# fenghansen/YOND_public

Measured on AMD Instinct MI355X. Metric: Bayer megapixels/sec end-to-end (NLE+VST+denoise+iVST), higher is better.
Workload: dtype f32 (3x3 convolutions: f32 operands as two f16 halves -- 22-23 significant bits -- on the f16 MFMA, 3 products per f32 product, f32 accumulate; per-layer error vs float64 asserted <= 2x the f32 direct kernel's and <= 2e-5 of max|ref| (tests/test_hip_conv.py; measured 1.3e-6 vs 1.5e-6), whole frame v

## Files before the change

include/yond_hip.h:

```cpp
#ifndef YOND_HIP_H
#define YOND_HIP_H

#include <stddef.h>
#include <stdint.h>

#ifdef __cplusplus
extern "C" {
#endif

#define YOND_OK 0
#define YOND_EINVAL (-1)
#define YOND_EUNSUPPORTED (-2)

#define YOND_ABI_VERSION 8
int yond_abi_version(void);

int yond_pack_vst_norm_f32(const float* bayer, int H, int W, float* out, int pad_l, int pad_r, int pad_t,
                           int pad_b, int mode, double scale, double gain, double sigma, double lo,
                           double hi, const double* lut_x, const float* lut_y, int lut_n, float* img_max,
                           void* stream);

int yond_pack_vst_norm_biaslut_f32(const float* bayer, int H, int W, float* out, int pad_l, int pad_r, int pad_t,
                                   int pad_b, double scale, double gain, double sigma, double lo, double hi,
                                   const double* lut_x, const double* lut_y, int lut_n, float* img_max, void* stream);
// ... 28 lines not shown
typedef struct YondConvDesc {
    const float* src0;
    const float* src1;
    int C0, C1;
    int N, H, W;
    int Ho, Wo;
    int Cout;
    int ksize;
    int stride;
    int shuffle;
    int pre_act;
    int post_act;
    float slope;
    const float* wpk;
    const float* escale;
    const float* eshift;
    int ebatch;
    const float* res;
    float* dst;
    int tn;
    int kc;
    int algo;
    const float* out4_w;
    const float* out4_b;
    const float* out4_x;
    const float* out4_ub;
    float* out4_dst;
    unsigned int* status;
    int in_fmt, out_fmt;
    int res_fmt;
    unsigned long long* clk;
    int tile_order;
    float* dst2;
} YondConvDesc;
#define YOND_STATUS_HALF_OVERFLOW 1u
#define YOND_FMT_NHWC_F32 0
#define YOND_FMT_SPLIT_PLANES 1
#define YOND_FMT_PLANES4 2
#define YOND_SP_PLANE_UNITS(H, W) ((((H) * (W)) + 8) / 8 * 8)
#define YOND_SP_BYTES(N, C, H, W) ((size_t)(N) * ((C) / 16) * 4 * (size_t)YOND_SP_PLANE_UNITS(H, W) * 16)
#define YOND_HP_BYTES(N, C, H, W) ((size_t)(N) * ((C) / 16) * 2 * (size_t)YOND_SP_PLANE_UNITS(H, W) * 16)

int yond_conv_config(int ksize, int stride, int cin, int cout, int shuffle, int N, int Ho, int Wo, int* tn, int* kc);
int yond_pack_conv_weight_f32(const float* w, int cout, int cin, int ksize, int tn, int kc, float* dst);
int yond_pack_conv_weight_split_f32(const float* w, int cout, int cin, int ksize, int tn, int kc, float* dst);
int yond_conv2d_f32(const YondConvDesc* desc, void* stream);

int yond_conv_wino_supported(int cin, int cout);
int yond_pack_conv_wino_weight_f32(const float* w, int cout, int cin, int tn, float* dst);

int yond_conv_split_supported(int ksize, int stride, int cin, int cout);
int yond_pack_conv_split_weight_f32(const float* w, int cout, int cin, int ksize, int tn, int parts, float* dst);
int yond_gemm_k1_stationary_supported(const YondConvDesc* desc);
int yond_pack_conv_split_weight_dev_f32(const float* w, int cout, int cin, int ksize, int tn, int parts, float* dst, int* status,
                                        void* stream);
int yond_pack_conv_split_weights_batch_dev_f32(const float* src, const long long* desc, int nlayers, float* dst, size_t ngroups,
                                               int* status, void* stream);

int yond_conv_in_f32(const float* x, const float* ub , int N, int H, int W, int Cout,
                     const float* wpk, const float* bias, float slope, float* dst,
                     int out_fmt , void* stream);
int yond_pack_conv_in_weight_f32(const float* w , int cout, float* dst );

int yond_conv_out_f32(const float* feat , int Cin, const float* w ,
                      const float* bias , const float* x ,
                      const float* ub , int N, int H, int W, float* dst ,
                      void* stream);

int yond_maxpool2_f32(const float* src, int N, int H, int W, int C, float* dst, void* stream);

typedef struct YondFilmDesc {
    int kind, C, ld;
    const float *w_a0, *b_a0, *w_a2, *b_a2;
    const float *w_b0, *b_b0;
    const float *w_b, *b_b;
    const float *cb1, *cb2;
    float *s1, *t1, *s2, *t2;
} YondFilmDesc;
int yond_film_f32(const YondFilmDesc* descs, int nblocks, const float* t , const float* ub ,
                  int N, void* stream);

int yond_box_stats_self1_f32(const float* bayer, int H, int W, int k, int k2, int tile_w, float* mean,
                             float* var, float* blur2, void* stream);
int yond_box_stats_self2_f32(const float* blur2, int h, int w, int k, int tile_w, float* lap, void* stream);
int yond_box_stats_collab_f32(const float* bayer_lr, const float* bayer_hr, int H, int W, int k, int tile_w,
                              float* mean, float* var, float* lap, void* stream);


int yond_box_stats_self_stats_f32(const float* bayer, int H, int W, int k, int k2, int tile_w, float* mean, float* var,
                                  float* blur2, float* lap, const double* q_host, int nq, void* ws, void* stream);
int yond_box_stats_collab_stats_f32(const float* bayer_lr, const float* bayer_hr, int H, int W, int k, int tile_w,
                                    float* mean, float* var, float* lap, const double* q_host, int nq, void* ws, void* stream);

size_t yond_select_ws_bytes(int nr);
int yond_select_ranks_f32(const float* data, size_t n, const int64_t* ranks_host, int nr, float* out, void* ws,
                          void* stream);
int yond_percentiles_f32(const float* data, size_t n, const double* q_host, int nq, double* out, void* ws,
                         void* stream);

size_t yond_nle_ws_bytes(size_t n);
int yond_nle_stats_f32(const float* lap, const float* mean, size_t n, int width, const double* q_host, int nq, void* ws,
                       void* stream);
int yond_nle_threshold_f32(const float* lap, size_t n, const double* q_host, int nq, int want_score, void* ws, void* stream);
int yond_nle_state_layout(int* off );
int yond_nle_moments_f32(const float* lap, const float* mean, const float* var, size_t n, void* ws, void* stream);

// ... 214 lines not shown
```

yond_public_amd/_lib.py:

```python
import ctypes as C
import os

import torch

_HERE = os.path.dirname(os.path.abspath(__file__))
LIB_PATH = os.environ.get("YOND_HIP_LIB", os.path.join(_HERE, "libyond_hip.so"))
_lib = None
ABI_VERSION = 8

vp, i32, f32, f64, sz, i64 = C.c_void_p, C.c_int, C.c_float, C.c_double, C.c_size_t, C.c_longlong


class YondConvDesc(C.Structure):
    _fields_ = [("src0", vp), ("src1", vp), ("C0", i32), ("C1", i32), ("N", i32), ("H", i32), ("W", i32),
                ("Ho", i32), ("Wo", i32), ("Cout", i32), ("ksize", i32), ("stride", i32), ("shuffle", i32),
                ("pre_act", i32), ("post_act", i32), ("slope", f32), ("wpk", vp), ("escale", vp),
                ("eshift", vp), ("ebatch", i32), ("res", vp), ("dst", vp), ("tn", i32), ("kc", i32), ("algo", i32),
                ("out4_w", vp), ("out4_b", vp), ("out4_x", vp), ("out4_ub", vp), ("out4_dst", vp), ("status", vp),
                ("in_fmt", i32), ("out_fmt", i32), ("res_fmt", i32), ("clk", vp), ("tile_order", i32), ("dst2", vp)]


class YondBlock0Desc(C.Structure):
    _fields_ = [("x", vp), ("in_fmt", i32), ("N", i32), ("H", i32), ("W", i32), ("w1", vp), ("w2", vp),
                ("s1", vp), ("t1", vp), ("s2", vp), ("t2", vp), ("ebatch", i32), ("dst", vp),
                ("out4_w", vp), ("out4_b", vp), ("out4_x", vp), ("out4_ub", vp), ("out4_dst", vp), ("status", vp)]


class YondFilmDesc(C.Structure):
    _fields_ = [("kind", i32), ("C", i32), ("ld", i32),
                ("w_a0", vp), ("b_a0", vp), ("w_a2", vp), ("b_a2", vp), ("w_b0", vp), ("b_b0", vp),
                ("w_b", vp), ("b_b", vp), ("cb1", vp), ("cb2", vp),
                ("s1", vp), ("t1", vp), ("s2", vp), ("t2", vp)]


PROTOTYPES = {
    "yond_abi_version": [],
    "yond_pack_vst_norm_f32": [vp, i32, i32, vp, i32, i32, i32, i32, i32, f64, f64, f64, f64, f64, vp, vp, i32, vp, vp],
    "yond_pack_vst_norm_biaslut_f32": [vp, i32, i32, vp, i32, i32, i32, i32, f64, f64, f64, f64, f64, vp, vp, i32, vp, vp],
    "yond_bias_eval_f32": [vp, sz, vp, vp, i32, i32, i32, f64, f64, vp, vp],
    "yond_denorm_ivst_unpack_f32": [vp, i32, i32, i32, i32, i32, i32, vp, i32, f64, f64, f64, f64, f64, i32, vp],
    "yond_pack_vst_norm_batch_f32": [vp, i32, i32, i32, vp, i32, i32, i32, i32, f64, f64, f64, f64, f64, vp, vp, i32, i32, vp, vp],
    "yond_denorm_ivst_unpack_batch_f32": [vp, i32, i32, i32, i32, i32, i32, i32, vp, i32, f64, f64, f64, f64, f64, i32, vp],
    "yond_vst_elem_f32": [vp, sz, f64, f64, f64, vp, vp],
    "yond_ivst_elem_f64": [vp, sz, f64, f64, i32, vp, vp],
    "yond_bayer2rggb_f32": [vp, i32, i32, vp, vp],
    "yond_rggb2bayer_f32": [vp, i32, i32, vp, vp],
    "yond_rot90_f32": [vp, i32, i32, i32, i32, vp, vp],
    "yond_nchw4_to_nhwc4_f32": [vp, vp, i32, i32, i32, vp],
    "yond_nhwc4_to_nchw4_f32": [vp, vp, i32, i32, i32, vp],
    "yond_image_max_f32": [vp, i32, sz, vp, vp, vp],
    "yond_conv_config": [i32, i32, i32, i32, i32, i32, i32, i32, C.POINTER(i32), C.POINTER(i32)],
    "yond_pack_conv_weight_f32": [vp, i32, i32, i32, i32, i32, vp],
    "yond_conv2d_f32": [C.POINTER(YondConvDesc), vp],
    "yond_conv_wino_supported": [i32, i32],
    "yond_pack_conv_wino_weight_f32": [vp, i32, i32, i32, vp],
    "yond_pack_conv_weight_split_f32": [vp, i32, i32, i32, i32, i32, vp],
    "yond_conv_split_supported": [i32, i32, i32, i32],
    "yond_pack_conv_split_weight_f32": [vp, i32, i32, i32, i32, i32, vp],
    "yond_gemm_k1_stationary_supported": [C.POINTER(YondConvDesc)],
    "yond_pack_conv_split_weight_dev_f32": [vp, i32, i32, i32, i32, i32, vp, vp, vp],
    "yond_pack_conv_split_weights_batch_dev_f32": [vp, vp, i32, vp, sz, vp, vp],
    "yond_conv_in_f32": [vp, vp, i32, i32, i32, i32, vp, vp, f32, vp, i32, vp],
    "yond_pack_conv_in_weight_f32": [vp, i32, vp],
    "yond_conv_out_f32": [vp, i32, vp, vp, vp, vp, i32, i32, i32, vp, vp],
    "yond_maxpool2_f32": [vp, i32, i32, i32, i32, vp, vp],
    "yond_film_f32": [vp, i32, vp, vp, i32, vp],
    "yond_box_stats_self1_f32": [vp, i32, i32, i32, i32, i32, vp, vp, vp, vp],
    "yond_box_stats_self2_f32": [vp, i32, i32, i32, i32, vp, vp],
    "yond_box_stats_collab_f32": [vp, vp, i32, i32, i32, i32, vp, vp, vp, vp],
    "yond_box_stats_self_stats_f32": [vp, i32, i32, i32, i32, i32, vp, vp, vp, vp, vp, i32, vp, vp],
    "yond_box_stats_collab_stats_f32": [vp, vp, i32, i32, i32, i32, vp, vp, vp, vp, i32, vp, vp],
    "yond_select_ws_bytes": [i32],
    "yond_select_ranks_f32": [vp, sz, vp, i32, vp, vp, vp],
    "yond_percentiles_f32": [vp, sz, vp, i32, vp, vp, vp],
    "yond_nle_ws_bytes": [sz],
    "yond_nle_stats_f32": [vp, vp, sz, i32, vp, i32, vp, vp],
    "yond_nle_threshold_f32": [vp, sz, vp, i32, i32, vp, vp],
    "yond_nle_state_layout": [vp],
    "yond_nle_moments_f32": [vp, vp, vp, sz, vp, vp],
    "yond_nlf_occupancy_f32": [vp, vp, sz, i32, vp, i32, vp, vp],
    "yond_nlf_score3_f64": [vp, vp, vp, i32, vp, vp, vp],
    "yond_nlf_moments_f32": [vp, vp, vp, sz, vp, vp, vp],
    "yond_bias_lut_f64": [vp, i32, f64, f64, vp, vp],
    "yond_block_metrics_tiles": [i32, i32],
    "yond_block_metrics_f32": [vp, vp, i32, i32, i32, i32, vp, vp],
    "yond_block_metrics_rgb8": [vp, vp, i32, i32, i32, i32, vp, vp],
    "yond_render_srgb": [vp, i32, i32, i32, i32, i32, C.POINTER(f64), C.POINTER(f64), i32, vp, vp, i32, vp, f64, vp],
    "yond_clock_probe": [f64, vp, vp],
    "yond_img2raw_f32": [vp, sz, i32, i32, i32, vp, vp, i32, i32, i32, vp, vp, vp, vp],
    "yond_pg_noise_f32": [vp, vp, sz, i32, vp, i32, vp],
    "yond_camera_noise_f32": [vp, vp, sz, i32, vp, i32, i32, vp],
    "yond_est_conv_in_f32": [vp, i32, i32, i32, i32, vp, vp, vp, vp],
    "yond_est_head_f32": [vp, i32, i32, i32, i32, vp, vp, i32, i32, i32, vp, vp, vp],
    "yond_est_head_ws_bytes": [i32, i32],
    "yond_conv_wgrad_f32": [vp, vp, i32, i32, i32, i32, i32, i32, i32, i32, i32, vp, vp],
    "yond_conv_wgrad_ws_f32": [vp, vp, i32, i32, i32, i32, i32, i32, i32, i32, i32, vp, vp, sz, vp],
    "yond_conv_wgrad_ws_bytes": [i32, i32, i32, i32, i32, i32, i32, i32, i32],
    "yond_conv_wgrad_split_ws_bytes": [i32, i32, i32, i32, i32],
    "yond_conv_wgrad_split_f32": [vp, vp, i32, i32, i32, i32, i32, vp, i32, vp, sz, vp, vp],
    "yond_colsum_f32": [vp, sz, i32, vp, vp],
    "yond_film_silu_supported": [i32],
    "yond_film_silu_f32": [vp, vp, vp, vp, i32, sz, i32, vp],
    "yond_film_silu_bwd_f32": [vp, vp, vp, vp, vp, vp, vp, i32, sz, i32, vp],
    "yond_film_mlp_fwd_f32": [vp, vp, vp, vp, vp, vp, vp, i32, i32, i32, vp, vp, vp],
    "yond_film_mlp_bwd_f32": [vp, vp, vp, vp, vp, vp, vp, vp, i32, i32, i32, vp, vp, vp, vp, vp, vp, vp, vp],
    "yond_film_mlp_fwd_multi_f32": [vp, i32, vp],
    "yond_gemm_split_f32": [vp, i32, sz, i32, i32, i64, i64, i32, vp, vp, i32, i32, i32, i32, vp, vp],
    "yond_film_mlp_bwd_multi_f32": [vp, i32, vp],
    "yond_silu_bwd_add_f32": [vp, vp, vp, vp, sz, vp],
    "yond_silu_f32": [vp, vp, sz, vp],
    "yond_zero_interleave_f32": [vp, i32, i32, i32, i32, i32, i32, vp, vp],
    "yond_l1_loss_f32": [vp, vp, sz, vp, vp, vp],
# ... 113 lines not shown
```

yond_public_amd/csrc/conv.hip:

```cpp
#include "common.h"
#include <cstdlib>

#ifndef YOND_B32_WGS
#define YOND_B32_WGS 2
#endif
#ifndef YOND_ABL
#define YOND_ABL 0
#endif

template <int KS, int STRIDE, int TH, int TN, int KC>
struct ConvCfg {
    static constexpr int TW = 32;
    static constexpr int TAPS = KS * KS;
    static constexpr int PADK = KS / 2;
    static constexpr int IH = (TH - 1) * STRIDE + KS;
    static constexpr int IW = (TW - 1) * STRIDE + KS;
    static constexpr int HALF = (IW + 1) / 2;
    static constexpr int TWP = (STRIDE == 2) ? 2 * HALF : IW;
    static constexpr int PS = KC + 4;
    static constexpr int IN_FLOATS = IH * TWP * PS;
    static constexpr int Q = KC / 8;
    static constexpr int W_FLOATS = TAPS * Q * 2 * TN * 4;
    static constexpr int BUF_FLOATS = IN_FLOATS + W_FLOATS;
    static constexpr int NW = TN / 32;
// ... 467 lines not shown
    {
        const long e11 = yond_exp_long("YOND_1X1_TN", 0), es2 = yond_exp_long("YOND_S2_TN", 0), ekc = yond_exp_long("YOND_CONV_KC", 0),
                   etn = yond_exp_long("YOND_CONV_TN", 0);
        if (e11 && ksize == 1) t = e11 == 32 ? 32 : (ntile % 64 == 0 ? 64 : 32);
        if (es2 && ksize == 3 && stride == 2) t = es2 == 32 ? 32 : (ntile % 64 == 0 ? 64 : 32);
        if (ekc && ksize == 3 && stride == 1) k = ekc == 8 ? 8 : 16;
        if (etn && ksize == 3 && stride == 1 && ntile % 64 == 0) t = etn == 32 ? 32 : 64;
    }
#endif
    if (tn) *tn = t;
    if (kc) *kc = k;
    return YOND_OK;
}

extern "C" int yond_pack_conv_weight_f32(const float* w, int cout, int cin, int ksize, int tn, int kc, float* dst) {
    if (!w || !dst || (tn != 32 && tn != 64) || cout % tn != 0 || cin % kc != 0 || kc % 8 != 0) return YOND_EINVAL;
    const int taps = ksize * ksize, Q = kc / 8;
    size_t o = 0;
    for (int ct = 0; ct < cout / tn; ++ct)
        for (int ch = 0; ch < cin / kc; ++ch)
            for (int tap = 0; tap < taps; ++tap)
                for (int q = 0; q < Q; ++q)
                    for (int h = 0; h < 2; ++h)
                        for (int j = 0; j < tn; ++j)
                            for (int e = 0; e < 4; ++e) {
                                const int co = ct * tn + j, ci = ch * kc + q * 8 + h * 4 + e;
                                dst[o++] = w[((size_t)co * cin + ci) * taps + tap];
                            }
    return YOND_OK;
}

extern "C" int yond_pack_conv_weight_split_f32(const float* w, int cout, int cin, int ksize, int tn, int kc, float* dst) {
    const int rc = yond_pack_conv_weight_f32(w, cout, cin, ksize, tn, kc, dst);
    if (rc != YOND_OK) return rc;
    const size_t n = (size_t)cout * cin * ksize * ksize;
    for (size_t i = 0; i < n; ++i)
        if (!(fabsf(w[i]) <= 65504.0f)) return YOND_EUNSUPPORTED;
    for (size_t i = 0; i < n; ++i) {
        const float v = dst[i];
        const _Float16 h = (_Float16)v;
        const _Float16 l = (_Float16)((v - (float)h) * 2048.0f);
        unsigned short hb, lb;
        __builtin_memcpy(&hb, &h, 2);
        __builtin_memcpy(&lb, &l, 2);
        const unsigned u = (unsigned)hb | ((unsigned)lb << 16);
        __builtin_memcpy(&dst[i], &u, 4);
    }
    return YOND_OK;
}

int yond_conv_wino_dispatch(const YondConvDesc& d, hipStream_t st);
int yond_conv_split_dispatch(const YondConvDesc& d, hipStream_t st);
int yond_gemm_k1_stationary_dispatch(const YondConvDesc& d, hipStream_t st);

extern "C" int yond_conv2d_f32(const YondConvDesc* dp, void* stream) {
    if (!dp) return YOND_EINVAL;
    const YondConvDesc& d = *dp;
    hipStream_t st = (hipStream_t)stream;
    if (!d.src0 || !(d.dst || d.out4_dst) || !d.wpk || d.N <= 0 || d.H <= 0 || d.W <= 0 || d.Ho <= 0 || d.Wo <= 0) return YOND_EINVAL;
    if (d.out4_dst && ((d.algo != 3 && d.algo != 4) || !d.out4_w || d.Cout != 32 || d.stride != 1)) return YOND_EUNSUPPORTED;
    if (d.C1 > 0 && !d.src1) return YOND_EINVAL;
    if (d.shuffle < 0 || d.shuffle > 2) return YOND_EINVAL;
    if (d.shuffle == 2 && d.algo != 3 && d.algo != 4 && d.algo != 6) return YOND_EUNSUPPORTED;
    if ((long long)d.N * d.H * d.W > 0x7fffffffLL) return YOND_EUNSUPPORTED;
    if (d.pre_act != 0 && d.pre_act != 1) return YOND_EINVAL;
    if (d.in_fmt < 0 || d.in_fmt > 2 || d.out_fmt < 0 || d.out_fmt > 2 || (d.res_fmt != 0 && d.res_fmt != 2)) return YOND_EINVAL;
    if (d.algo == 6) return yond_gemm_k1_stationary_dispatch(d, st);
    if ((d.in_fmt || d.out_fmt || d.res_fmt) && d.algo != 3 && d.algo != 4) return YOND_EUNSUPPORTED;
    if (d.algo == 1) return yond_conv_wino_dispatch(d, st);
    if (d.algo == 3 || d.algo == 4) return yond_conv_split_dispatch(d, st);
    if (d.algo != 0 && d.algo != 2 && d.algo != 5) return YOND_EINVAL;
    if (d.tn != 32 && d.tn != 64) return YOND_EINVAL;
    int tn, kc;
    const int rc = yond_conv_config(d.ksize, d.stride, d.C0 + d.C1, d.Cout, d.shuffle, 0, 0, 0, &tn, &kc);
    if (rc != YOND_OK) return rc;
    tn = d.tn;
    if (d.kc != 0) kc = d.kc;
    if (kc != 8 && kc != 16) return YOND_EINVAL;
    if (kc == 8 && d.ksize != 3) return YOND_EINVAL;
    if (d.ksize == 3 && d.stride == 2 && kc != 8) return YOND_EINVAL;
    if (d.C0 % kc != 0 || d.C1 % kc != 0 || d.Cout % tn != 0) return YOND_EUNSUPPORTED;
    if (d.shuffle && (d.ksize != 1 || (d.Cout / 4) % tn != 0)) return YOND_EUNSUPPORTED;
    if ((long long)d.N * d.H * d.W > 0x7fffffffLL) return YOND_EUNSUPPORTED;
    if (d.stride == 2) {
        if (d.Ho != (d.H + 1) / 2 || d.Wo != (d.W + 1) / 2) return YOND_EINVAL;
    } else if (d.Ho != d.H || d.Wo != d.W) return YOND_EINVAL;
    if (d.pre_act != 0 && d.pre_act != 1) return YOND_EINVAL;
    if (d.post_act != 0 && d.post_act != 2) return YOND_EUNSUPPORTED;
    if (d.pre_act == 1 && !(d.ksize == 3 && d.stride == 1)) return YOND_EUNSUPPORTED;
    if (d.ksize == 3 && d.stride == 1 && kc == 8) {
        if (d.pre_act) return tn == 64 ? launch_conv<3, 1, 8, 64, 8, true>(d, st) : launch_conv<3, 1, 8, 32, 8, true>(d, st);
        return tn == 64 ? launch_conv<3, 1, 8, 64, 8, false>(d, st) : launch_conv<3, 1, 8, 32, 8, false>(d, st);
    }
    if (d.ksize == 3 && d.stride == 1) {
        if (d.pre_act) return tn == 64 ? launch_conv<3, 1, 8, 64, 16, true>(d, st) : launch_conv<3, 1, 8, 32, 16, true>(d, st);
        return tn == 64 ? launch_conv<3, 1, 8, 64, 16, false>(d, st) : launch_conv<3, 1, 8, 32, 16, false>(d, st);
    }
    if (d.ksize == 3 && d.stride == 2)
        return tn == 64 ? launch_conv<3, 2, 8, 64, 8, false>(d, st) : launch_conv<3, 2, 4, 32, 8, false>(d, st);
    return tn == 64 ? launch_conv<1, 1, 8, 64, 16, false>(d, st) : launch_conv<1, 1, 8, 32, 16, false>(d, st);
}
```

yond_public_amd/engine.py:

```python
import ctypes as C
import os

import numpy as np
import torch

from . import _lib as L


def _rup(c, m=32):
    return (c + m - 1) // m * m


def _np_ptr(a):
    return C.c_void_p(a.ctypes.data)


FILM_MAX_C = 1024


WINO_DEFAULT = 'split'


SPLIT_PLANES = True
SP_FLOW = True
HALF_FLOW = True
HALF_K1_TN128 = True
HALF_S2_TN128 = True
HALF_FLOW_TN128 = True
HALF_TN128 = True
FUSE_OUT4 = True
FUSE_BLOCK0 = False
K1_SUB2 = True
K1_D2_LEVELS = (3,)
K1_STATIONARY_LEVELS = (2, 1, 0)
K1_D2_LEVELS_HALF = ()
SP_CONV1_MIN_LEVEL = 3
UNET_SP = True
SNAKE_ORDER = True


def sp_plane_units(H, W):
    return (H * W + 8) // 8 * 8


class _PackedConv:

    def __init__(self, dev, weight, bias, ksize, stride, splits, shuffle=False):
        lib = L.load()
        w = weight.detach().to('cpu', torch.float32).numpy()
        if shuffle:
            cin, cout = w.shape[0], w.shape[1]
            coutp = _rup(cout)
            m = np.zeros((4, coutp, cin), np.float32)
            m[:, :cout, :] = w.transpose(2, 3, 1, 0).reshape(4, cout, cin)
            w = m.reshape(4 * coutp, cin, 1, 1)
            self.cout_real_p = coutp
            gemm_n = 4 * coutp
        else:
            cout = w.shape[0]
            coutp = _rup(cout)
            gemm_n = coutp
            self.cout_real_p = coutp
        assert sum(splits) == w.shape[1], (splits, w.shape)
        psplits = [_rup(s) for s in splits]
        cinp = sum(psplits)
        wp = np.zeros((gemm_n, cinp, ksize, ksize), np.float32)
        so, do = 0, 0
        for s, ps in zip(splits, psplits):
            wp[:w.shape[0], do:do + s] = w[:, so:so + s]
            so += s
            do += ps
        self._wp = np.ascontiguousarray(wp)
        self._packed = {}
        self._dev = dev
        b = torch.zeros(coutp, dtype=torch.float32)
        if bias is not None:
            b[:cout] = bias.detach().to('cpu', torch.float32)
        self.bias = b.to(dev)
        self.ksize, self.stride, self.shuffle = ksize, stride, shuffle
        self.psplits, self.gemm_n, self.coutp, self.cinp = psplits, gemm_n, coutp, cinp
        self.cin_real, self.cout_real = sum(splits), cout
        self.config(0, 0, 0)
        self.wmax = float(np.abs(self._wp).max()) if self._wp.size else 0.0
        self.macs_per_pixel = self.cin_real * self.cout_real * (4 if shuffle else ksize * ksize)

    def config(self, N, Ho, Wo, split=False):
        lib = L.load()
# ... 237 lines not shown
            d.Ho, d.Wo = H, W
        d.Cout = pc.gemm_n
        d.ksize, d.stride, d.shuffle = pc.ksize, pc.stride, int(pc.shuffle)
        d.pre_act, d.post_act, d.slope = pre_act, post_act, slope
        prec = getattr(self, 'precision', 'fp32')
        if getattr(self, 'strict', False) and algo is None:
            prec, algo = 'fp32-mfma', 1
        if algo is None:
            algo = getattr(self, 'conv_algo', WINO_DEFAULT)
            if prec == 'fp32-mfma' and algo == 'split':
                algo = 1
            if prec == 'fp16' and WINO_DEFAULT == 'split':
                algo = 'half'
        fp16 = prec == 'fp16' or algo == 'fp16'
        wino = split = None
        if algo in ('split', 'half'):
            ws2 = (HALF_S2_TN128 and algo == 'half' and pc.stride == 2 and in_fmt == 1 and out_fmt == 2 and dst2 is None
                   and (pc.gemm_n // 128) * ((d.Wo + 31) // 32) * ((d.Ho + 7) // 8) * N >= 256)
            ws2 = ws2 or (HALF_K1_TN128 and algo == 'half' and pc.ksize == 1 and in_fmt == 1 and dst2 is None)
            split = pc.split(2 if algo == 'split' else 1, wide=(not (in_fmt or out_fmt or res_fmt or dst2 is not None)) or (HALF_FLOW_TN128 and out_fmt == 1),
                             wide_s2=ws2)
            if algo == 'half' and pc.ksize == 1 and in_fmt != 1:
                split = None
            if split is None and not fp16 and pc.ksize == 3:
                wino = pc.wino()
        elif not fp16:
            wino = pc.wino() if algo in (1, 2) else None
        if split is not None:
            tn, wpk = split
            kc = 16
            d.algo = 3 if algo == 'split' else 4
        elif wino is not None:
            tn, wpk = wino
            kc = 8
            d.algo = 1
        elif algo == 'split' and pc.ksize == 1 and not fp16 and pc.config(N, d.Ho, d.Wo, split=True)[2] is not None:
            tn, kc, wpk = pc.config(N, d.Ho, d.Wo, split=True)
            d.algo = 5
        else:
            tn, kc, wpk = pc.config(N, d.Ho, d.Wo)
            d.algo = 2 if (fp16 and pc.wmax <= 65504.0) else 0
        d.wpk = wpk.data_ptr()
        d.tn = tn
        d.kc = kc
        d.escale = escale.data_ptr() if escale is not None else None
        d.eshift = (eshift if eshift is not None else pc.bias).data_ptr()
        d.ebatch = ebatch
        d.res = res.data_ptr() if res is not None else None
        d.dst = dst.data_ptr() if dst is not None else None
        status = getattr(self, 'status', None)
        d.status = status.data_ptr() + 4 * self.status_slot if status is not None else None
        d.in_fmt, d.out_fmt, d.res_fmt = in_fmt, out_fmt, res_fmt
        d.dst2 = dst2.data_ptr() if dst2 is not None else None
        if stationary and d.algo == 3 and self.lib.yond_gemm_k1_stationary_supported(C.byref(d)):
            d.algo = 6
        if SNAKE_ORDER and d.algo in (3, 4, 6):
            self._tile_order = 1 - getattr(self, '_tile_order', 0)
            d.tile_order = self._tile_order
        clk = getattr(self, 'clk', None)
        d.clk = clk.data_ptr() if (clk is not None and d.algo in (3, 4, 6)) else None
        if (in_fmt or out_fmt or res_fmt) and d.algo not in (3, 4, 6):
            raise L.YondHipError("split-plane / 4-channel-plane tensors need the split-operand kernel (algo 3, or 4 with h-only planes)")
        if out4 is not None:
            w4, b4, x4, ub4, o4 = out4
            if d.algo not in (3, 4):
                raise L.YondHipError("fused output projection needs the split-operand 3x3 kernel")
            d.out4_w, d.out4_b = w4.data_ptr(), (b4.data_ptr() if b4 is not None else None)
            d.out4_x = x4.data_ptr() if x4 is not None else None
            d.out4_ub = ub4.data_ptr() if ub4 is not None else None
            d.out4_dst = o4.data_ptr()
        prof = getattr(self, 'prof', None)
        if prof is not None:
            tag = f"conv_wino_kernel<{tn}>" if d.algo == 1 else f"conv_mfma_kernel<{pc.ksize},{pc.stride},8,{tn},{kc}>"
            if d.algo in (3, 4, 6):
                tag = f"conv_split_kernel<{pc.stride if pc.ksize == 3 else 'k1'},{tn},{1 if d.algo == 4 else 2}>" + ("/stationary" if d.algo == 6 else "")
            if d.algo == 2:
                tag += "/f16"
            if d.algo == 5:
                tag += "/split"
            only = getattr(self, 'prof_only', None)
            if only is not None and not only(tag):
                prof = None
            every = getattr(self, 'prof_every', 1)
            if every > 1 and getattr(self, '_fwd_idx', 0) % every:
                prof = None
        if prof is not None:
            e0, e1 = torch.cuda.Event(enable_timing=True), torch.cuda.Event(enable_timing=True)
            e0.record()
        L.check(self.lib.yond_conv2d_f32(C.byref(d), L.stream()), "yond_conv2d_f32")
        if prof is not None:
            e1.record()
            prof.append((tag, 2.0 * pc.macs_per_pixel * N * d.Ho * d.Wo, e0, e1))
        return dst

    def _block0_weights(self, pc):
        w = getattr(pc, '_b0', None)
        if w is None:
            if not L.has("yond_pack_block0_weight_f32"):
                raise L.YondHipError("the fused level-0 block exists only in experiment builds of the library (python -m yond_public_amd.build --experiments)")
            if not (pc.ksize == 3 and pc.stride == 1 and pc.gemm_n == 32 and pc.cinp == 32 and len(pc.psplits) == 1):
                return None
            host = np.zeros(9 * 2 * 4 * 32 * 8, np.float16)
            if self.lib.yond_pack_block0_weight_f32(_np_ptr(pc._wp), 32, 32, _np_ptr(host)) != 0:
                return None
            w = pc._b0 = torch.from_numpy(host.view(np.float32)).to(pc._dev)
        return w

    def _block0(self, pc1, pc2, x, N, H, W, f, in_fmt, dst=None, out4=None):
        w1, w2 = self._block0_weights(pc1), self._block0_weights(pc2)
        d = L.YondBlock0Desc()
        d.x, d.in_fmt, d.N, d.H, d.W = x.data_ptr(), in_fmt, N, H, W
        d.w1, d.w2 = w1.data_ptr(), w2.data_ptr()
        d.s1, d.t1, d.s2, d.t2 = (None if v is None else v.data_ptr() for v in f)
        d.ebatch = 1
        d.dst = dst.data_ptr() if dst is not None else None
        if out4 is not None:
            w4, b4, x4, ub4, o4 = out4
            d.out4_w, d.out4_b = w4.data_ptr(), (b4.data_ptr() if b4 is not None else None)
            d.out4_x = x4.data_ptr() if x4 is not None else None
            d.out4_ub = ub4.data_ptr() if ub4 is not None else None
            d.out4_dst = o4.data_ptr()
        status = getattr(self, 'status', None)
        d.status = status.data_ptr() + 4 * self.status_slot if status is not None else None
        prof = getattr(self, 'prof', None)
        if prof is not None:
            tag = "block0_fused_kernel" + ("<o4>" if out4 is not None else "")
            only = getattr(self, 'prof_only', None)
            if (only is not None and not only(tag)) or (getattr(self, 'prof_every', 1) > 1 and getattr(self, '_fwd_idx', 0) % getattr(self, 'prof_every', 1)):
# ... 100 lines not shown
                    xs = self._new(N, 2 * h, 2 * w, cp)
                    up = blk['upsc2'] if (flow and K1_SUB2 and 'upsc2' in blk) else blk['upsc']
                    xsp = (self._new_sp(('xspd', i), N, 2 * h, 2 * w, cp, pt)
                           if (flow and not last and (9 - i) in (K1_D2_LEVELS if pt == 2 else K1_D2_LEVELS_HALF) and up is blk['upsc'] and cp % 64 == 0 and w > 16) else None)
                    self._conv(up, cur, skips[10 - i], N, h, w, xs, in_fmt=SP if flow else 0, out_fmt=xfmt, dst2=xsp,
                               stationary=(9 - i) in K1_STATIONARY_LEVELS)
                    h, w = 2 * h, 2 * w
                    cur = xs
                if flow and FUSE_BLOCK0 and h == H and cp == 32 and self._block0_weights(blk['conv1']) is not None and self._block0_weights(blk['conv2']) is not None:
                    if last and self._out4_fusable(blk['conv2'], flow):
                        out4 = self._new(N, H, W, 4)
                        self._block0(blk['conv1'], blk['conv2'], cur, N, h, w, f, xfmt, out4=(self.w_out, self.b_out, x4 if self.res else None, ub, out4))
                        return out4
                    if not last:
                        out = self._new_sp(('out', i), N, h, w, cp, pt)
                        self._block0(blk['conv1'], blk['conv2'], cur, N, h, w, f, xfmt, dst=out)
                        cur = out
                        skips[i] = cur
                        nxt = self._new(N, h // 2, w // 2, blk['pool'].coutp)
                        xsp = self._new_sp(('xsp', i + 1), N, h // 2, w // 2, blk['pool'].coutp, pt) if (flow and i >= SP_CONV1_MIN_LEVEL) else None
                        self._conv(blk['pool'], cur, None, N, h, w, nxt, in_fmt=SP, out_fmt=P4, dst2=xsp)
                        h, w = h // 2, w // 2
                        cur = nxt
                        continue
                act_in_producer = self._split_pair(blk['conv1'], blk['conv2'])
                sp = SP if (flow or (act_in_producer and SPLIT_PLANES and getattr(self, 'precision', 'fp32') == 'fp32'
                                      and sp_plane_units(h, w) * 64 < 2 ** 31)) else 0
                tmp = self._new_sp(('tmp', i), N, h, w, cp, pt) if sp else self._new(N, h, w, cp)
                if xsp is not None and sp and act_in_producer:
                    self._conv(blk['conv1'], xsp, None, N, h, w, tmp, escale=f[0], eshift=f[1], ebatch=1, pre_act=0, post_act=1,
                               in_fmt=SP, out_fmt=sp)
                else:
                    self._conv(blk['conv1'], cur, None, N, h, w, tmp, escale=f[0], eshift=f[1], ebatch=1, pre_act=1,
                               post_act=1 if act_in_producer else 0, in_fmt=xfmt, out_fmt=sp)
                xsp = None
                pre2 = 0 if act_in_producer else 1
                if last and self._out4_fusable(blk['conv2'], flow):
                    out4 = self._new(N, H, W, 4)
                    self._conv(blk['conv2'], tmp, None, N, h, w, None, escale=f[2], eshift=f[3], ebatch=1, res=cur, pre_act=pre2,
                               out4=(self.w_out, self.b_out, x4 if self.res else None, ub, out4), in_fmt=sp)
                    return out4
                if flow:
                    out = self._new_sp(('out', i), N, h, w, cp, pt)
                    self._conv(blk['conv2'], tmp, None, N, h, w, out, escale=f[2], eshift=f[3], ebatch=1, res=cur, pre_act=pre2,
                               in_fmt=SP, out_fmt=SP, res_fmt=P4)
                else:
                    out = self._new(N, h, w, cp)
                    self._conv(blk['conv2'], tmp, None, N, h, w, out, escale=f[2], eshift=f[3], ebatch=1, res=cur, pre_act=pre2, in_fmt=sp)
                cur = out
                if i <= 4:
                    skips[i] = cur
                    nxt = self._new(N, h // 2, w // 2, blk['pool'].coutp)
                    xsp = self._new_sp(('xsp', i + 1), N, h // 2, w // 2, blk['pool'].coutp, pt) if (flow and i >= SP_CONV1_MIN_LEVEL) else None
                    self._conv(blk['pool'], cur, None, N, h, w, nxt, in_fmt=SP if flow else 0, out_fmt=P4 if flow else 0, dst2=xsp)
                    h, w = h // 2, w // 2
                    cur = nxt
            feat = cur
        else:
            a = self._new(N, H, W, nfp)
            L.check(lib.yond_conv_in_f32(L.ptr(x4), L.ptr(ub), N, H, W, nfp, L.ptr(self.conv_in_w), L.ptr(self.conv_in_b),
                                         0.2, L.ptr(a), 0, st), "yond_conv_in_f32")
            cv = self.convs
            h, w = H, W
            cur = self._conv(cv['conv1_2'], a, None, N, h, w, self._new(N, h, w, cv['conv1_2'].coutp), post_act=2, slope=0.2)
            skips = {1: cur}

            def first_of_pair(i, c1, c2, s0, s1):
                sp = (UNET_SP and SPLIT_PLANES and not getattr(self, 'strict', False) and getattr(self, 'conv_algo', WINO_DEFAULT) == 'split'
                      and getattr(self, 'precision', 'fp32') == 'fp32' and c1.split(2) is not None and c2.split(2) is not None
                      and N * sp_plane_units(h, w) * 64 < 2 ** 31)
                dst = self._new_sp(('utmp', i), N, h, w, c1.coutp) if sp else self._new(N, h, w, c1.coutp)
                self._conv(c1, s0, s1, N, h, w, dst, post_act=2, slope=0.2, out_fmt=1 if sp else 0)
                return dst, (1 if sp else 0)

            for i in range(2, 6):
                cpv = cur.shape[-1]
                pooled = self._new(N, h // 2, w // 2, cpv)
                L.check(lib.yond_maxpool2_f32(L.ptr(cur), N, h, w, cpv, L.ptr(pooled), st), "yond_maxpool2_f32")
                h, w = h // 2, w // 2
                c1, c2 = cv[f'conv{i}_1'], cv[f'conv{i}_2']
                cur, fmt = first_of_pair(i, c1, c2, pooled, None)
                cur = self._conv(c2, cur, None, N, h, w, self._new(N, h, w, c2.coutp), post_act=2, slope=0.2, in_fmt=fmt)
                if i < 5:
                    skips[i] = cur
            for i in range(6, 10):
                upc = cv[f'upv{i}']
                up = self._new(N, 2 * h, 2 * w, upc.cout_real_p)
                self._conv(upc, cur, None, N, h, w, up)
                h, w = 2 * h, 2 * w
                c1, c2 = cv[f'conv{i}_1'], cv[f'conv{i}_2']
                cur, fmt = first_of_pair(i, c1, c2, up, skips[10 - i])
                if i == 9 and self._out4_fusable(c2):
                    out4 = self._new(N, H, W, 4)
                    self._conv(c2, cur, None, N, h, w, None, post_act=2, slope=0.2, in_fmt=fmt,
                               out4=(self.w_out, self.b_out, x4 if self.res else None, ub, out4))
                    return out4
                cur = self._conv(c2, cur, None, N, h, w, self._new(N, h, w, c2.coutp), post_act=2, slope=0.2, in_fmt=fmt)
            feat = cur
        out4 = self._new(N, H, W, 4)
        L.check(lib.yond_conv_out_f32(L.ptr(feat), feat.shape[-1], L.ptr(self.w_out), L.ptr(self.b_out),
                                      L.ptr(x4) if self.res else None, L.ptr(ub), N, H, W, L.ptr(out4), st), "yond_conv_out_f32")
        return out4

    def forward_nchw(self, x, t=None):
        L.require_cuda(x, "x")
        N, c, H, W = x.shape
        if c != 4:
# ... 28 lines not shown
```

Before: 2662.

## Add weight-stationary stride-2 3x3 conv kernel for level-2 pool layer

```diff
diff --git a/include/yond_hip.h b/include/yond_hip.h
--- a/include/yond_hip.h
+++ b/include/yond_hip.h
@@ -104,6 +104,7 @@
 int yond_conv_split_supported(int ksize, int stride, int cin, int cout);
 int yond_pack_conv_split_weight_f32(const float* w, int cout, int cin, int ksize, int tn, int parts, float* dst);
 int yond_gemm_k1_stationary_supported(const YondConvDesc* desc);
+int yond_conv3_stationary_supported(const YondConvDesc* desc);
 int yond_pack_conv_split_weight_dev_f32(const float* w, int cout, int cin, int ksize, int tn, int parts, float* dst, int* status,
                                         void* stream);
 int yond_pack_conv_split_weights_batch_dev_f32(const float* src, const long long* desc, int nlayers, float* dst, size_t ngroups,
diff --git a/yond_public_amd/_lib.py b/yond_public_amd/_lib.py
--- a/yond_public_amd/_lib.py
+++ b/yond_public_amd/_lib.py
@@ -58,6 +58,7 @@
     "yond_conv_split_supported": [i32, i32, i32, i32],
     "yond_pack_conv_split_weight_f32": [vp, i32, i32, i32, i32, i32, vp],
     "yond_gemm_k1_stationary_supported": [C.POINTER(YondConvDesc)],
+    "yond_conv3_stationary_supported": [C.POINTER(YondConvDesc)],
     "yond_pack_conv_split_weight_dev_f32": [vp, i32, i32, i32, i32, i32, vp, vp, vp],
     "yond_pack_conv_split_weights_batch_dev_f32": [vp, vp, i32, vp, sz, vp, vp],
     "yond_conv_in_f32": [vp, vp, i32, i32, i32, i32, vp, vp, f32, vp, i32, vp],
diff --git a/yond_public_amd/csrc/conv.hip b/yond_public_amd/csrc/conv.hip
--- a/yond_public_amd/csrc/conv.hip
+++ b/yond_public_amd/csrc/conv.hip
@@ -543,6 +543,7 @@
 int yond_conv_wino_dispatch(const YondConvDesc& d, hipStream_t st);
 int yond_conv_split_dispatch(const YondConvDesc& d, hipStream_t st);
 int yond_gemm_k1_stationary_dispatch(const YondConvDesc& d, hipStream_t st);
+int yond_conv3_stationary_dispatch(const YondConvDesc& d, hipStream_t st);
 
 extern "C" int yond_conv2d_f32(const YondConvDesc* dp, void* stream) {
     if (!dp) return YOND_EINVAL;
@@ -557,6 +558,7 @@
     if (d.pre_act != 0 && d.pre_act != 1) return YOND_EINVAL;
     if (d.in_fmt < 0 || d.in_fmt > 2 || d.out_fmt < 0 || d.out_fmt > 2 || (d.res_fmt != 0 && d.res_fmt != 2)) return YOND_EINVAL;
     if (d.algo == 6) return yond_gemm_k1_stationary_dispatch(d, st);
+    if (d.algo == 7) return yond_conv3_stationary_dispatch(d, st);
     if ((d.in_fmt || d.out_fmt || d.res_fmt) && d.algo != 3 && d.algo != 4) return YOND_EUNSUPPORTED;
     if (d.algo == 1) return yond_conv_wino_dispatch(d, st);
     if (d.algo == 3 || d.algo == 4) return yond_conv_split_dispatch(d, st);
diff --git a/yond_public_amd/csrc/conv3_stationary.hip b/yond_public_amd/csrc/conv3_stationary.hip
--- /dev/null
+++ b/yond_public_amd/csrc/conv3_stationary.hip
@@ -0,0 +1,207 @@
+#include "common.h"
+
+typedef _Float16 f16x8 __attribute__((ext_vector_type(8)));
+typedef unsigned u32x4 __attribute__((ext_vector_type(4)));
+
+template <int NCH, int D>
+__global__ __launch_bounds__(512) void conv3_stationary_kernel(const YondConvDesc d) {
+    constexpr int NCOL = NCH * 3;
+    constexpr int CHF = 9 * 1024;
+    static_assert(NCOL % D == 0 && D >= 2 && (NCH * 9) % 2 == 0, "the ring holds whole rounds of a segment's columns; the two fragment sets close at its end");
+    constexpr int FILM_OFF = NCH * CHF;
+    constexpr int STRIDE = 2;
+    extern __shared__ __attribute__((aligned(16))) float smem[];
+    const int tid = threadIdx.x, lane = tid & 63, wave = __builtin_amdgcn_readfirstlane(tid >> 6);
+    const int li = lane & 31, lh = lane >> 5;
+    const int nct = d.Cout / 64;
+    const int per_xcd = gridDim.x / 8;
+    const int bx = blockIdx.x % 8, bj = blockIdx.x / 8;
+    const int ct = bj % nct, grp = bx * (per_xcd / nct) + bj / nct, ngrp = gridDim.x / nct;
+    const bool clk_on = d.clk != nullptr && blockIdx.x == 0 && tid == 0;
+    const unsigned long long clk_c0 = __builtin_amdgcn_s_memtime(), clk_r0 = __builtin_amdgcn_s_memrealtime();
+
+    {
+        const f32x4* wsrc = (const f32x4*)(d.wpk + (size_t)ct * NCH * CHF);
+        f32x4* wl = (f32x4*)smem;
+        for (int i = tid; i < NCH * CHF / 4; i += 512) wl[i] = wsrc[i];
+        float* film = smem + FILM_OFF;
+        const int nfilm = d.ebatch ? d.N : 1;
+        for (int i = tid; i < nfilm * 128; i += 512) {
+            const int im = i >> 7, k = i & 127;
+            const int cb = ct * 64 + (k & 63);
+            film[i] = k < 64 ? (d.escale ? d.escale[im * d.Cout + cb] : 1.0f) : (d.eshift ? d.eshift[im * d.Cout + cb] : 0.0f);
+        }
+    }
+    __syncthreads();
+
+    const int nsx = (d.Wo + 31) / 32, nyb = (d.Ho + 7) / 8;
+    const int nband = d.N * nyb * nsx;
+    if (grp < nband) {
+        const bool rev = d.tile_order != 0;
+        const unsigned PS = (unsigned)YOND_SP_PLANE_UNITS(d.H, d.W) * 16u;
+        const unsigned zoff = (unsigned)lh * 2u * PS + (unsigned)(d.H * d.W) * 16u;
+        const unsigned hw_out = (unsigned)(d.Ho * d.Wo);
+        const float slope_eff = d.post_act == 2 ? d.slope : 1.0f;
+        struct Geo { int n, y, x; unsigned base, vr, vc; };
+        auto geo = [&](int s) {
+            Geo g;
+            const int t = rev ? nband - 1 - s : s;
+            const int per = nyb * nsx;
+            g.n = t / per;
+            const int r = t - g.n * per;
+            const int yb = r / nsx;
+            g.y = yb * 8 + wave;
+            g.x = (r - yb * nsx) * 32 + li;
+            const int iy = STRIDE * g.y - 1, ix = STRIDE * g.x - 1;
+            g.base = (unsigned)lh * 2u * PS + (unsigned)(iy * d.W + ix) * 16u;
+            g.vr = g.vc = 0;
+#pragma unroll
+            for (int k = 0; k < 3; ++k) {
+                g.vr |= (iy + k >= 0 && iy + k < d.H ? 1u : 0u) << k;
+                g.vc |= (ix + k >= 0 && ix + k < d.W ? 1u : 0u) << k;
+            }
+            return g;
+        };
+        f16x8 ring[D][3][2];
+        auto issue = [&](auto cc, const Geo& g) __attribute__((always_inline)) {
+            constexpr int c = decltype(cc)::value, slot = c % D, ch = c / 3, dx = c % 3;
+            const char* b = (const char*)d.src0 + ((size_t)g.n * NCH + ch) * 4 * (size_t)PS;
+#pragma unroll
+            for (int dy = 0; dy < 3; ++dy) {
+                const bool in = ((g.vr >> dy) & (g.vc >> dx) & 1u) != 0;
+                const unsigned v = in ? g.base + (unsigned)(dy * d.W + dx) * 16u : zoff;
+                ring[slot][dy][0] = *(const f16x8*)(b + v);
+                ring[slot][dy][1] = *(const f16x8*)(b + PS + v);
+            }
+        };
+        typedef const __attribute__((address_space(3))) f16x8* lds_h8;
+        const __attribute__((address_space(3))) float* wb = (const __attribute__((address_space(3))) float*)(smem + (lh * 2 * 64 + li) * 4);
+        const float* film = smem + FILM_OFF;
+        const __amdgpu_buffer_rsrc_t orsrc = __builtin_amdgcn_make_buffer_rsrc(d.dst, 0, (int)((unsigned)d.N * (unsigned)d.Cout * hw_out * 4u), 0x00020000);
+        f16x8 wt[2][2][2];
+        auto load_w = [&](auto jc) __attribute__((always_inline)) {
+            constexpr int j = decltype(jc)::value, c = j / 3, dy = j % 3, ch = c / 3, dx = c % 3, tap = dy * 3 + dx;
+#pragma unroll
+            for (int nn = 0; nn < 2; ++nn)
+#pragma unroll
+                for (int p = 0; p < 2; ++p) wt[j % 2][nn][p] = *(lds_h8)(wb + ch * CHF + ((tap * 4 + p) * 64 + nn * 32) * 4);
+        };
+
+        auto segment = [&](const Geo& cur, const Geo& nxt) __attribute__((always_inline)) {
+            f32x16 acc[2][2];
+#pragma unroll
+            for (int a = 0; a < 2; ++a)
+#pragma unroll
+                for (int nn = 0; nn < 2; ++nn)
+#pragma unroll
+                    for (int r = 0; r < 16; ++r) acc[a][nn][r] = 0.0f;
+            const bool ok = cur.x < d.Wo && cur.y < d.Ho;
+            const unsigned OUT = 0x80000000u;
+            const unsigned pix = (unsigned)(cur.y * d.Wo + cur.x);
+            static_for<0, NCOL>([&](auto cc) __attribute__((always_inline)) {
+                constexpr int c = decltype(cc)::value, slot = c % D;
+                static_for<0, 3>([&](auto yc) __attribute__((always_inline)) {
+                    constexpr int dy = decltype(yc)::value, j = c * 3 + dy, ws = j % 2;
+                    load_w(IntC<(j + 1) % (NCOL * 3)>{});
+                    const f16x8 xh = ring[slot][dy][0], xl = ring[slot][dy][1];
+#pragma unroll
+                    for (int nn = 0; nn < 2; ++nn) acc[1][nn] = __builtin_amdgcn_mfma_f32_32x32x16_f16(wt[ws][nn][0], xl, acc[1][nn], 0, 0, 0);
+#pragma unroll
+                    for (int nn = 0; nn < 2; ++nn) acc[0][nn] = __builtin_amdgcn_mfma_f32_32x32x16_f16(wt[ws][nn][0], xh, acc[0][nn], 0, 0, 0);
+#pragma unroll
+                    for (int nn = 0; nn < 2; ++nn) acc[1][nn] = __builtin_amdgcn_mfma_f32_32x32x16_f16(wt[ws][nn][1], xh, acc[1][nn], 0, 0, 0);
+                });
+                if constexpr (c + D < NCOL) issue(IntC<c + D>{}, cur);
+                else issue(IntC<c + D - NCOL>{}, nxt);
+                __builtin_amdgcn_sched_barrier(0);
+            });
+            const float* fv = film + (d.ebatch ? cur.n * 128 : 0) + 4 * lh;
+#pragma unroll
+            for (int nn = 0; nn < 2; ++nn) {
+                const unsigned ob = ok ? ((unsigned)(cur.n * (d.Cout / 4) + ct * 16 + nn * 8 + lh) * hw_out + pix) * 16u : OUT;
+#pragma unroll
+                for (int g = 0; g < 4; ++g) {
+                    const f32x4 es = *(const f32x4*)(fv + nn * 32 + 8 * g), et = *(const f32x4*)(fv + 64 + nn * 32 + 8 * g);
+                    f32x4 v;
+#pragma unroll
+                    for (int e = 0; e < 4; ++e) {
+                        float x = acc[0][nn][4 * g + e];
+                        x = fmaf(acc[1][nn][4 * g + e], 1.0f / 2048.0f, x);
+                        x = fmaf(x, es[e], et[e]);
+                        x = x > 0.0f ? x : x * slope_eff;
+                        v[e] = x + 0.0f;
+                    }
+                    __builtin_amdgcn_raw_buffer_store_b128(__builtin_bit_cast(u32x4, v), orsrc, (int)(ob + (unsigned)g * 32u * hw_out), 0, 0);
+                }
+            }
+        };
+
+        const long long sstep = ngrp;
+        Geo cur = geo(grp);
+        static_for<0, D>([&](auto cc) { issue(cc, cur); });
+        load_w(IntC<0>{});
+        long long sn = grp + sstep;
+        Geo nxt = sn < nband ? geo((int)sn) : cur;
+        segment(cur, nxt);
+        while (sn < nband) {
+            cur = nxt;
+            sn += sstep;
+            nxt = sn < nband ? geo((int)sn) : cur;
+            segment(cur, nxt);
+        }
+        asm volatile("s_waitcnt vmcnt(0)" ::: "memory");
+    }
+    if (clk_on) {
+        atomicAdd(d.clk, __builtin_amdgcn_s_memtime() - clk_c0);
+        atomicAdd(d.clk + 1, __builtin_amdgcn_s_memrealtime() - clk_r0);
+    }
+}
+
+static int c3s_chunks(const YondConvDesc& d) {
+    if (d.ksize != 3 || d.stride != 2 || d.shuffle != 0 || d.tn != 64 || !d.src0 || d.src1 || d.C1 || !d.dst || !d.wpk) return 0;
+    if (d.in_fmt != YOND_FMT_SPLIT_PLANES || d.dst2 || d.out4_dst || d.pre_act) return 0;
+    if (d.C0 != 32 && d.C0 != 64) return 0;
+    if (d.N <= 0 || d.H <= 0 || d.W <= 0 || d.Cout <= 0 || d.Cout % 64) return 0;
+    const int nct = d.Cout / 64;
+    if (32 % nct) return 0;
+    if (d.ebatch && d.N > 16) return 0;
+    if (d.Ho != (d.H + 1) / 2 || d.Wo != (d.W + 1) / 2 || d.out_fmt != YOND_FMT_PLANES4 || d.res || d.res_fmt) return 0;
+    if (d.post_act != 0 && d.post_act != 2) return 0;
+    if ((long long)d.N * d.Cout * d.Ho * d.Wo * 4 >= 0x7fffffffLL) return 0;
+    if ((long long)d.N * ((d.Ho + 7) / 8) * ((d.Wo + 31) / 32) > 0x7fffffffLL) return 0;
+    if ((long long)YOND_SP_PLANE_UNITS(d.H, d.W) * 4 * 16 * 4 >= 0x7fffffffLL) return 0;
+    return d.C0 / 16;
+}
+
+extern "C" int yond_conv3_stationary_supported(const YondConvDesc* d) { return (d && (d->algo == 3 || d->algo == 7) && c3s_chunks(*d)) ? 1 : 0; }
+
+template <int NCH, int D>
+static int launch_c3s(const YondConvDesc& d, hipStream_t st) {
+    constexpr int SMEM = (NCH * 9 * 1024 + 16 * 128) * 4;
+    static_assert(SMEM <= 160 * 1024, "LDS budget");
+    static bool attr_set = false;
+    auto kern = conv3_stationary_kernel<NCH, D>;
+    if (!attr_set) {
+        hipError_t e = hipFuncSetAttribute((const void*)kern, hipFuncAttributeMaxDynamicSharedMemorySize, SMEM);
+        if (e != hipSuccess) return (int)e;
+        attr_set = true;
+    }
+    constexpr int C3S_GRID = 256;
+    static_assert(C3S_GRID % 8 == 0, "whole XCD shares");
+    hipLaunchKernelGGL(kern, dim3(C3S_GRID), dim3(512), SMEM, st, d);
+    YOND_LAUNCH_CHECK();
+    return YOND_OK;
+}
+
+int yond_conv3_stationary_dispatch(const YondConvDesc& d, hipStream_t st) {
+    const int nch = c3s_chunks(d);
+#ifdef YOND_EXPERIMENTS
+    const long depth = yond_exp_long("YOND_C3S_DEPTH", 0);
+    if (nch == 4 && depth == 3) return launch_c3s<4, 3>(d, st);
+    if (nch == 2 && depth == 2) return launch_c3s<2, 2>(d, st);
+    if (nch == 2 && depth == 6) return launch_c3s<2, 6>(d, st);
+#endif
+    if (nch == 4) return launch_c3s<4, 4>(d, st);
+    if (nch == 2) return launch_c3s<2, 3>(d, st);
+    return YOND_EUNSUPPORTED;
+}
diff --git a/yond_public_amd/engine.py b/yond_public_amd/engine.py
--- a/yond_public_amd/engine.py
+++ b/yond_public_amd/engine.py
@@ -33,6 +33,7 @@
 K1_SUB2 = True
 K1_D2_LEVELS = (3,)
 K1_STATIONARY_LEVELS = (2, 1, 0)
+C3_STATIONARY_LAYERS = (('pool', 2),)
 K1_D2_LEVELS_HALF = ()
 SP_CONV1_MIN_LEVEL = 3
 UNET_SP = True
@@ -376,14 +377,16 @@
         d.status = status.data_ptr() + 4 * self.status_slot if status is not None else None
         d.in_fmt, d.out_fmt, d.res_fmt = in_fmt, out_fmt, res_fmt
         d.dst2 = dst2.data_ptr() if dst2 is not None else None
-        if stationary and d.algo == 3 and self.lib.yond_gemm_k1_stationary_supported(C.byref(d)):
+        if stationary and d.algo == 3 and pc.ksize == 1 and self.lib.yond_gemm_k1_stationary_supported(C.byref(d)):
             d.algo = 6
-        if SNAKE_ORDER and d.algo in (3, 4, 6):
+        if stationary and d.algo == 3 and pc.ksize == 3 and self.lib.yond_conv3_stationary_supported(C.byref(d)):
+            d.algo = 7
+        if SNAKE_ORDER and d.algo in (3, 4, 6, 7):
             self._tile_order = 1 - getattr(self, '_tile_order', 0)
             d.tile_order = self._tile_order
         clk = getattr(self, 'clk', None)
-        d.clk = clk.data_ptr() if (clk is not None and d.algo in (3, 4, 6)) else None
-        if (in_fmt or out_fmt or res_fmt) and d.algo not in (3, 4, 6):
+        d.clk = clk.data_ptr() if (clk is not None and d.algo in (3, 4, 6, 7)) else None
+        if (in_fmt or out_fmt or res_fmt) and d.algo not in (3, 4, 6, 7):
             raise L.YondHipError("split-plane / 4-channel-plane tensors need the split-operand kernel (algo 3, or 4 with h-only planes)")
         if out4 is not None:
             w4, b4, x4, ub4, o4 = out4
@@ -396,8 +399,8 @@
         prof = getattr(self, 'prof', None)
         if prof is not None:
             tag = f"conv_wino_kernel<{tn}>" if d.algo == 1 else f"conv_mfma_kernel<{pc.ksize},{pc.stride},8,{tn},{kc}>"
-            if d.algo in (3, 4, 6):
-                tag = f"conv_split_kernel<{pc.stride if pc.ksize == 3 else 'k1'},{tn},{1 if d.algo == 4 else 2}>" + ("/stationary" if d.algo == 6 else "")
+            if d.algo in (3, 4, 6, 7):
+                tag = f"conv_split_kernel<{pc.stride if pc.ksize == 3 else 'k1'},{tn},{1 if d.algo == 4 else 2}>" + ("/stationary" if d.algo == 6 else "/stationary/c3" if d.algo == 7 else "")
             if d.algo == 2:
                 tag += "/f16"
             if d.algo == 5:
@@ -604,7 +607,8 @@
                     skips[i] = cur
                     nxt = self._new(N, h // 2, w // 2, blk['pool'].coutp)
                     xsp = self._new_sp(('xsp', i + 1), N, h // 2, w // 2, blk['pool'].coutp, pt) if (flow and i >= SP_CONV1_MIN_LEVEL) else None
-                    self._conv(blk['pool'], cur, None, N, h, w, nxt, in_fmt=SP if flow else 0, out_fmt=P4 if flow else 0, dst2=xsp)
+                    self._conv(blk['pool'], cur, None, N, h, w, nxt, in_fmt=SP if flow else 0, out_fmt=P4 if flow else 0, dst2=xsp,
+                               stationary=('pool', i) in C3_STATIONARY_LAYERS)
                     h, w = h // 2, w // 2
                     cur = nxt
             feat = cur
```

Measured after the change: 2652. No clear change (-0.4%).
